# Banksylel/Restrictive-Hierarchical-Semantic-Segmentation

Hardware: AMD Instinct MI355X
Metric: train images/sec (620x620, hier-HRNet-W48) (higher is better)
Workload: dtype f32 (fp16x2 split on fp16 MFMA, 22-bit operands, fp32 accumulate; exact-fp32 MFMA on the small problems); 1 GPU; HRNet-W48 hierarchical (class_tree_tl.json), 620x620, batch 4 per GPU, train_epoch batch body (fwd L passes, prediction prep + metrics, CE+Dice+consistency, bwd, grad all-reduce, AdamW, metric vectors, one D2H readback of loss+metrics); global_batch=4, parallelism=dp1, launch=launch tape replay, rccl_ranks=1, level_passes=batched (one launch per layer for all L passes)

## Files before the change

### include/hrseg.h

```cpp
#ifndef HRSEG_H
#define HRSEG_H

#include <stddef.h>
#include <stdint.h>

#ifdef __cplusplus
extern "C" {
#endif

typedef void* hrseg_stream_t;

enum hrseg_status {
  HRSEG_OK = 0,
  HRSEG_ERR_INVALID_ARG = -1,
  HRSEG_ERR_LAUNCH = -2,
  HRSEG_ERR_UNSUPPORTED = -3,
};

const char* hrseg_last_error_string(void);
int hrseg_abi_version(void);

enum hrseg_conv_precision { HRSEG_CONV_F32 = 0, HRSEG_CONV_BF16X3 = 1, HRSEG_CONV_BF16X2 = 2, HRSEG_CONV_BF16 = 3, HRSEG_CONV_AUTO = 4,
                            HRSEG_CONV_FP16X2 = 5 };
typedef struct {
// ... 121 lines not shown
int hrseg_head_bn_fwd(const float* y, int ldy, const float* coef, const float* gb, const float* w, const float* bias,
                      float* z, int ldz, int B, long hw, int F, int Cout, hrseg_stream_t stream);
#define HRSEG_HEAD_BN_MAX_SEG 8
typedef struct {
  const float* y; int ldy; const float* coef;
  int F, nseg, B; long hw;
  double* partial; int nchunks;
  float* dy_absmax;
  float* dy; int lddy;
  const float* gb[HRSEG_HEAD_BN_MAX_SEG]; const float* w[HRSEG_HEAD_BN_MAX_SEG];
  const float* dzl[HRSEG_HEAD_BN_MAX_SEG]; int lddzl[HRSEG_HEAD_BN_MAX_SEG]; int Cout[HRSEG_HEAD_BN_MAX_SEG];
  float* dw[HRSEG_HEAD_BN_MAX_SEG]; float* dbias[HRSEG_HEAD_BN_MAX_SEG]; float* dgb[HRSEG_HEAD_BN_MAX_SEG];
} hrseg_head_bn_t;
int hrseg_head_bn_bwd_reduce(const hrseg_head_bn_t* p, int seg0, int nsegs, hrseg_stream_t stream);
int hrseg_head_bn_bwd_apply(const hrseg_head_bn_t* p, hrseg_stream_t stream);
int hrseg_logits_up_fwd(const float* in, int ldin, int B, int Hi, int Wi, int C, float* out, int Ho,
                        int Wo, int align_corners, hrseg_stream_t stream);
int hrseg_logits_up_bwd(const float* dout, int B, int Hi, int Wi, int C, float* din, int lddin,
                        int Ho, int Wo, int align_corners, hrseg_stream_t stream);

int hrseg_sigmoid_fwd(const float* z, float* p, long n, hrseg_stream_t stream);
int hrseg_compose_fwd(const float* z, const float* pprev, float* p, int B, int C, int Cprev,
                      long hw, int ngroups, const int* group_parent, const int* group_size,
                      hrseg_stream_t stream);
int hrseg_compose_bwd(const float* dp, long sb, long sc, long si, const float* z,
                      const float* pprev, float* dz, int dz_accumulate, float* dpprev,
                      int dpprev_accumulate, int B, int C, int Cprev, long hw, int ngroups,
                      const int* group_parent, const int* group_size, hrseg_stream_t stream);
int hrseg_sigmoid_bwd(const float* dp, long sb, long sc, long si, const float* z, float* dz,
                      int accumulate, int B, int C, long hw, hrseg_stream_t stream);
// ... 226 lines not shown
```

### restrictive-hierarchical-semantic-segmentation_amd/_lib.py

```python
from __future__ import annotations

import ctypes as C
import os

import torch

_HERE = os.path.dirname(os.path.abspath(__file__))
LIB_PATH = os.path.join(_HERE, "csrc", "libhrseg_hip.so")

if not os.path.exists(LIB_PATH):
    raise ImportError(
        f"{LIB_PATH} not found: the MI355X HIP library is not built. "
        "Run `make -C restrictive-hierarchical-semantic-segmentation_amd/csrc` (needs hipcc); "
        "there is no CPU fallback for the product path.")

_lib = C.CDLL(LIB_PATH)

_p = C.c_void_p
_i = C.c_int
_l = C.c_long
_f = C.c_float


class ConvShape(C.Structure):
# ... 9 lines not shown
                ("running_var", _p), ("num_batches_tracked", _p), ("momentum", _f), ("eps", _f), ("residual", _p),
                ("ldr", _i), ("relu", _i), ("z", _p), ("ldz", _i), ("coef", _p), ("partial", _p), ("nchunks", _i),
                ("stat_div", _i), ("stat_updates", _i), ("relu_mask", _p), ("z_split", _i), ("residual_split", _i), ("stat_ranks", _i)]


class BnBwd(C.Structure):
    _fields_ = [("dz", _p), ("lddz", _i), ("z", _p), ("ldz", _i), ("relu", _i), ("y", _p), ("ldy", _i), ("coef", _p),
                ("dgamma", _p), ("dbeta", _p), ("dy", _p), ("lddy", _i), ("dres", _p), ("lddres", _i),
                ("dres_accumulate", _i), ("npix", _l), ("C", _i), ("partial", _p), ("nchunks", _i), ("dy_absmax", _p), ("nseg", _i), ("relu_mask", _p), ("sum_ranks", _i)]


class HeadBn(C.Structure):
    _fields_ = [("y", _p), ("ldy", _i), ("coef", _p), ("F", _i), ("nseg", _i), ("B", _i), ("hw", _l), ("partial", _p),
                ("nchunks", _i), ("dy_absmax", _p), ("dy", _p), ("lddy", _i), ("gb", _p * 8), ("w", _p * 8), ("dzl", _p * 8),
                ("lddzl", _i * 8), ("Cout", _i * 8), ("dw", _p * 8), ("dbias", _p * 8), ("dgb", _p * 8)]


class DecodeTree(C.Structure):
    _fields_ = [("first_child", (_i * 16) * 8), ("n_children", (_i * 16) * 8), ("pixel_val", (_i * 16) * 8), ("root_softmax", _i)]


class Hedge(C.Structure):
    _fields_ = [("tau", (_f * 16) * 8), ("stop_val", (_i * 16) * 8), ("reject_val", _i)]


PROTOTYPES = {
    "hrseg_conv_fwd_group": [_i, _p, _p, _p, _p, C.POINTER(ConvShape), _p],
    "hrseg_conv_dgrad_group": [_i, _p, _p, _p, _p, C.POINTER(ConvShape), _p],
    "hrseg_conv_wgrad_group": [_i, _p, _p, _p, C.POINTER(ConvShape), _p],
    "hrseg_conv_wgrad_group_ws": [_i, _p, _p, _p, C.POINTER(ConvShape), _p, C.c_size_t, _p],
# ... 15 lines not shown
    "hrseg_weight_cols_gather": [_p, _i, _i, _i, _p, _p, _p],
    "hrseg_weight_cols_scatter_add": [_p, _i, _i, _i, _p, _p, _p],
    "hrseg_add": [_p, _i, _p, _i, _p, _i, _i, _l, _i, _p],
    "hrseg_copy": [_p, _i, _p, _i, _i, _l, _i, _p],
    "hrseg_relu_bwd": [_p, _i, _p, _i, _p, _i, _l, _i, _p],
    "hrseg_nchw_to_nhwc": [_p, _p, _i, _i, _i, _i, _i, _p],
    "hrseg_nhwc_to_nchw": [_p, _i, _p, _i, _i, _i, _i, _p],
    "hrseg_gap_nchw": [_p, _p, _p, _i, _l, _p],
    "hrseg_film_linear_fwd": [_p, _p, _p, _p, _i, _i, _i, _p],
    "hrseg_film_linear_bwd": [_p, _p, _p, _p, _p, _p, _i, _i, _i, _f, _p],
    "hrseg_head_fwd": [_p, _i, _p, _p, _p, _p, _i, _i, _l, _i, _i, _p],
    "hrseg_head_bwd": [_p, _i, _p, _p, _p, _i, _p, _i, _i, _p, _p, _p, _i, _l, _i, _i, _p],
    "hrseg_head_bn_fwd": [_p, _i, _p, _p, _p, _p, _p, _i, _i, _l, _i, _i, _p],
    "hrseg_head_bn_bwd_reduce": [C.POINTER(HeadBn), _i, _i, _p],
    "hrseg_head_bn_bwd_apply": [C.POINTER(HeadBn), _p],
    "hrseg_logits_up_fwd": [_p, _i, _i, _i, _i, _i, _p, _i, _i, _i, _p],
    "hrseg_logits_up_bwd": [_p, _i, _i, _i, _i, _p, _i, _i, _i, _i, _p],
    "hrseg_sigmoid_fwd": [_p, _p, _l, _p],
    "hrseg_sigmoid_bwd": [_p, _l, _l, _l, _p, _p, _i, _i, _i, _l, _p],
    "hrseg_compose_fwd": [_p, _p, _p, _i, _i, _i, _l, _i, _p, _p, _p],
    "hrseg_compose_bwd": [_p, _l, _l, _l, _p, _p, _p, _i, _p, _i, _i, _i, _i, _l, _i, _p, _p, _p],
    "hrseg_loss_partials": [_p, _p, _p, _i, _i, _l, _p],
    "hrseg_loss_finalize": [_p, _p, _i, _i, _p, _p, _p],
    "hrseg_loss_bwd": [_p, _p, _p, _p, _p, _i, _i, _i, _l, _p],
    "hrseg_loss_partials_opt": [_p, _p, _p, _i, _i, _l, _f, _p],
    "hrseg_loss_finalize_opt": [_p, _p, _i, _i, _f, _f, _f, _p, _p, _p],
    "hrseg_loss_bwd_opt": [_p, _p, _p, _p, _p, _i, _i, _i, _l, _f, _p],
    "hrseg_ohem_scores": [_p, _p, _p, _i, _i, _l, _p],
    "hrseg_ohem_select": [_p, _l, _f, _l, _p, _p, _p],
    "hrseg_loss_partials_ohem": [_p, _p, _p, _p, _f, _p, _i, _i, _l, _f, _p],
# ... 133 lines not shown
def launch_count(family=None, reset=False) -> int:
    return int(_lib.hrseg_launch_count(None if family is None else family.encode(), int(reset)))


def deterministic() -> bool:
    return _deterministic


_fuse_bwd_multi = True


def fuse_bwd_multi() -> bool:
    return _fuse_bwd_multi


_tune_generation = 0


def tune_generation() -> int:
    return _tune_generation


def tune(**kv):
    global _deterministic, _fuse_bwd_multi, _tune_generation
    _tune_generation += 1
    for k, v in kv.items():
        if _lib.hrseg_tune(k.encode(), int(v)) != 0:
            raise RuntimeError(f"hrseg_tune({k}) failed: {last_error()}")
        if k == "deterministic":
            _deterministic = bool(v)
        if k == "fuse_bwd_multi":
            _fuse_bwd_multi = bool(v)


def set_conv_tune(wtm=0, kc=0, db=0, ksplit=0):
    tune(igemm_wtm=wtm, igemm_kc=kc, igemm_db=db, igemm_ksplit=ksplit)


def set_wgrad_tune(pix=0, db=0, target_blocks=0):
    tune(wgrad_pix=pix, wgrad_db=db, wgrad_blocks=target_blocks)


def set_wgrad_group_plan(mult=0, min_blocks=0, max_blocks=0):
    tune(wgrad_group_mult=mult, wgrad_group_min=min_blocks, wgrad_group_max=max_blocks)


_fn = {}
# ... 207 lines not shown
```

### restrictive-hierarchical-semantic-segmentation_amd/csrc/bn.hip

```cpp
#include <type_traits>
#include "elem_common.h"
#include "sp_arith.h"

__device__ __forceinline__ void reduce_chunks16(const double* __restrict__ partial, int nchunks, int C, int c,
                                               double& s0, double& s1, double* red) {
  const int lane = threadIdx.x >> 4;
  double a = 0.0, b = 0.0;
  if (c < C) {
    int k = lane;
    for (; k + 48 < nchunks; k += 64) {
      double t0[4], t1[4];
#pragma unroll
      for (int u = 0; u < 4; ++u) {
        t0[u] = partial[((size_t)(k + 16 * u) * 2 + 0) * C + c];
        t1[u] = partial[((size_t)(k + 16 * u) * 2 + 1) * C + c];
      }
#pragma unroll
      for (int u = 0; u < 4; ++u) {
        a += t0[u];
        b += t1[u];
      }
    }
    for (; k < nchunks; k += 16) {
      a += partial[((size_t)k * 2 + 0) * C + c];
// ... 767 lines not shown
}

extern "C" int hrseg_bn_bwd_group(int n, const hrseg_bn_bwd_t* probs, int eval_mode, hrseg_stream_t stream) {
  return hrseg_bn_bwd_group_phases(n, probs, eval_mode, 7, stream);
}

extern "C" int hrseg_bn_bwd_group_phases(int n, const hrseg_bn_bwd_t* probs, int eval_mode, int phases, hrseg_stream_t stream) {
  HRSEG_CHECK_ARG(n >= 1 && n <= BN_MAXG && probs, "hrseg_bn_bwd_group: n must be 1..%d", BN_MAXG);
  HRSEG_CHECK_ARG(phases > 0 && phases <= 7, "hrseg_bn_bwd_group_phases: phases is a mask of bits 0..2");
  hipStream_t st = (hipStream_t)stream;
  BnBwdG g;
  g.h.n = n;
  for (int i = 0; i < n; ++i) {
    const hrseg_bn_bwd_t& p = probs[i];
    if (int e = check_c(p.C, "hrseg_bn_bwd_group")) return e;
    HRSEG_CHECK_ARG(p.dz && p.y && p.coef && p.dy && p.partial && p.npix > 0 && p.nchunks > 0,
                    "hrseg_bn_bwd_group: bad arguments");
    HRSEG_CHECK_ARG(p.nseg <= 1 || (p.nchunks % p.nseg == 0 && p.npix % p.nseg == 0),
                    "hrseg_bn_bwd_group: nseg=%d must divide nchunks=%d and npix", p.nseg, p.nchunks);
    if (int e = check_operand(p.dz, p.lddz, p.C, "hrseg_bn_bwd_group", "dz")) return e;
    if (int e = check_operand(p.y, p.ldy, p.C, "hrseg_bn_bwd_group", "y")) return e;
    if (int e = check_operand(p.dy, p.lddy, p.C, "hrseg_bn_bwd_group", "dy")) return e;
    if (p.relu && p.z)
      if (int e = check_operand(p.z, p.ldz, p.C, "hrseg_bn_bwd_group", "z")) return e;
    if (p.dres)
      if (int e = check_operand(p.dres, p.lddres, p.C, "hrseg_bn_bwd_group", "dres")) return e;
    HRSEG_CHECK_ARG(al16(p.coef), "hrseg_bn_bwd_group: coef must be 16-byte aligned");
    g.p[i] = p;
  }
  int end = 0;
  bool masked = false;
  for (int i = 0; i < n; ++i) masked = masked || (probs[i].relu && probs[i].relu_mask);
  if (phases & 1) {
    for (int i = 0; i < n; ++i) { end += probs[i].nchunks; g.h.blk_end[i] = end; }
    if (masked) hipLaunchKernelGGL(bn_bwd_reduce_group_kernel<true>, dim3(end), dim3(256), 0, st, g);
    else hipLaunchKernelGGL(bn_bwd_reduce_group_kernel<false>, dim3(end), dim3(256), 0, st, g);
    HRSEG_LAUNCH_CHECK("bn_bwd_reduce_group");
  }
  if (phases & 2) {
    end = 0;
    for (int i = 0; i < n; ++i) { end += ceil_div(probs[i].C, 16); g.h.blk_end[i] = end; }
    hipLaunchKernelGGL(bn_bwd_finalize_group_kernel, dim3(end), dim3(256), 0, st, g);
// ... 71 lines not shown
```

### restrictive-hierarchical-semantic-segmentation_amd/csrc/runtime.h

```cpp
#pragma once

#define HRSEG_FAMILIES(X)                   \
  X(WS, "ws", 1)                            \
  X(WS_GROUP, "ws_group", 1)                \
  X(PATCH_SP, "patch_sp", 1)                \
  X(SP_IM2COL, "sp_im2col", 1)              \
  X(SP_PGROUP, "sp_pgroup", 1)              \
  X(SP_GROUP, "sp_group", 1)                \
  X(F32, "f32", 1)                          \
  X(F32_GROUP, "f32_group", 1)              \
  X(WGRAD_SP, "wgrad_sp", 1)                \
  X(WGRAD_F32, "wgrad_f32", 1)              \
  X(WGRAD_F32_GROUP, "wgrad_f32_group", 1)  \
  X(WGRAD9, "wgrad9", 1)                    \
  X(SMALL_CIN, "small_cin", 1)              \
  X(SP_WIDE, "sp_wide", 1)                  \
  X(WS_CANVAS, "ws_canvas", 0)              \
  X(WGRAD_SP_GROUP, "wgrad_sp_group", 1)    \
  X(WGRAD_SP_T5, "wgrad_sp_t5", 0)          \
  X(WGRAD_SP_WIDE, "wgrad_sp_wide", 1)      \
  X(AUG_IMAGE, "augment_image", 0)          \
  X(AUG_TARGETS, "augment_targets", 0)      \
  X(DECODE_LABELS, "decode_labels", 0)      \
  X(SCORE_LABELS, "score_labels", 0)        \
  X(DECODE_VIEWS, "decode_views", 0)        \
  X(FLIP_VIEWS, "flip_views", 0)          \
  X(WINDOW_CROPS, "window_crops", 0)      \
  X(DECODE_WINDOWS, "decode_windows", 0)  \
  X(OHEM, "ohem", 0)                      \
  X(LABEL_COMPONENTS, "label_components", 0)  \
  X(FILTER_COMPONENTS, "filter_components", 0)  \
  X(SCORE_BOUNDARIES, "score_boundaries", 0)  \
  X(SCORE_INSTANCES, "score_instances", 0)  \
  X(SCORE_CALIBRATION, "score_calibration", 0)  \
  X(DECODE_HEDGED, "decode_hedged", 0)  \
  X(MIX, "mix", 0)  \
  X(BORDER_WEIGHTS, "border_weights", 0)
#define HRSEG_X(id, name, conv) CNT_##id,
enum { HRSEG_FAMILIES(HRSEG_X) CNT_N };
#undef HRSEG_X
extern long hrseg_g_cnt[CNT_N];
static inline void hrseg_count(int id, long n = 1) { hrseg_g_cnt[id] += n; }

#define HRSEG_KNOBS(X)                                                                                                               \
  X(igemm_wtm, 0, 0, "fp32 implicit GEMM: pixel tiles per wave (1, 2, 4; +10 = 96-channel tiles)")                                   \
  X(igemm_kc, 0, 0, "fp32 implicit GEMM: 16-channel chunks per K stage")                                                             \
  X(igemm_db, 0, 0, "fp32 implicit GEMM: LDS buffers")                                                                               \
  X(igemm_ksplit, 0, 0, "fp32 implicit GEMM: split-K factor")                                                                        \
  X(group_wtm, 0, 0, "grouped launches: pixel tile, 1 = 64, 2 = 128 pixels")                                                         \
  X(wgrad_pix, 0, 0, "weight gradient: pixels per stage")                                                                            \
  X(wgrad_db, 0, 0, "weight gradient: LDS buffers")                                                                                  \
  X(wgrad_blocks, 0, 0, "weight gradient: target grid")                                                                              \
// ... 22 lines not shown
  X(wgrad9_blocks2, 0, 0, "  ... of two")                                                                                            \
  X(wgrad9_blocks3, 0, 0, "  ... of three")                                                                                          \
  X(wgrad9_blocks4, 0, 0, "  ... of four")                                                                                           \
  X(sp_wide, 1, 0, "0 = never use the wide-tile im2col body, 2 = also on short reductions (tests)")                                  \
  X(sp_ws_canvas, 5, 0, "canvas tiling of small images: least cut of the padded area, percent (0 = per-image tiles everywhere)")     \
  X(wgrad_group_sp, 1, 0, "0 = grouped tap-per-block weight gradients stay on the fp32 kernel")                                      \
  X(wgrad_sp_t5, 1, 0, "0 = no 80 x 80 tiles in the tap-per-block weight gradient")                                                  \
  X(wgrad_sp_wide, 1, 0, "0 = never the wide-tile weight-gradient body")                                                             \
  X(sp_wide_min_blocks, 256, 0, "wide-tile im2col body: least number of 128-pixel blocks")                                           \
  X(sp_patch_min_tiles, 192, 1, "routing threshold: least tile count of the halo-patch body")                                        \
  X(auto_min_pixels, 8192, 1, "routing threshold: HRSEG_CONV_AUTO runs fp16x2 from this many output pixels on")                      \
  X(sp_ws_min_tiles, 96, 1, "routing threshold: least tile count of the wave-specialised body")                                      \
  X(deterministic, 0, 0, "1 = every float reduction with a run-dependent order takes its single-adder form (common.h)")             \
  X(bwd_multi_slab, 0, 0, "multi-target bilinear transpose: channels of a slab of the streaming body (0 = automatic, < 0 = the gather body)") \
  X(bwd_multi_bands, 0, 0, "  ... its bands of target rows per image (0 = automatic; clamped to the coarsest target's rows)")        \
  X(fuse_bwd_multi, 1, 0, "0 = the fuse layers' backward transposes each low-resolution term in a launch of its own (engine.py)")
#define HRSEG_X(key, def, restore, meaning) extern int hrseg_g_##key;
HRSEG_KNOBS(HRSEG_X)
#undef HRSEG_X
```

### restrictive-hierarchical-semantic-segmentation_amd/engine.py

```python
from __future__ import annotations

import contextlib
import os

import torch

from . import _lib, ops

_SIDE = {}


_SIDE_ENABLED = None
_RELU_MASK = os.environ.get("HRSEG_BN_RELU_MASK", "1") != "0"
_EXPERIMENT = set(filter(None, os.environ.get("HRSEG_EXPERIMENT", "").split(",")))
_CONV_STATS = os.environ.get("HRSEG_CONV_STATS", "1") != "0"
_X_SPLIT = int(os.environ.get("HRSEG_X_SPLIT", "2"))


def wgrad_stream(device):
    global _SIDE_ENABLED
    if _SIDE_ENABLED is None:
        _SIDE_ENABLED = os.environ.get("HRSEG_WGRAD_STREAM", "1") != "0"
    if not _SIDE_ENABLED:
        return None
# ... 197 lines not shown
                                  split_for=[split_for] if split_for is not None else None, defer=defer)[0]

    def conv_bn_group(self, items, relu, outs=None, single_reader=False, split_for=None, split_level=1, defer=False):
        n = len(items)
        relus = list(relu) if isinstance(relu, (list, tuple)) else [relu] * n
        k, s = items[0][1].kernel_size[0], items[0][1].stride[0]
        assert all(c.kernel_size[0] == k and c.stride[0] == s for _, c, _, _ in items)
        xs = [it[0] for it in items]
        if not self.training and not self.record and self.fold is not None:
            folded = [self.fold(conv, bn) for _, conv, bn, _ in items]
            res = [it[3].data if it[3] is not None else None for it in items]
            prec = self.prec if all(f[2] for f in folded) else _lib.CONV_PRECISION["f32"]
            zs = ops.conv_fwd_group([x.data for x in xs], [f[0] for f in folded], [f[1] for f in folded], k, s,
                                    [c.out_channels for _, c, _, _ in items], prec=prec, residuals=res, relus=relus, outs=outs)
            return [Act(z) for z in zs]
        want_stats = self.training and _CONV_STATS and self.sync is None and not _lib.deterministic() and not _EXPERIMENT
        stats = None
        ys = ops.conv_fwd_group([x.data for x in xs], [c.weight._hr_store for _, c, _, _ in items],
                                [c.bias._hr_store if c.bias is not None else None for _, c, _, _ in items], k, s,
                                [c.out_channels for _, c, _, _ in items], prec=self.prec, stats=want_stats,
                                wpersist=self.wpersist, x_splits=[x.split for x in xs])
        if want_stats:
            ys, stats = ys
        if stats is not None and any(st is None for st in stats):
            stats = None

        def conv_backward(dys, gmax_all, gmaxs):
            def weight_gradients():
                if "skip_wgrad" in _EXPERIMENT:
                    return
# ... 10 lines not shown
            while todo:
                seen, rnd, rest = set(), [], []
                for i in todo:
                    (rest if id(xs[i]) in seen else rnd).append(i)
                    seen.add(id(xs[i]))
                wp = self.wpersist and all(hasattr(items[i][1].weight, "_hr_tstore_range") for i in rnd)
                got = ops.conv_dgrad_group([dys[i] for i in rnd], [self._wt(items[i][1]) for i in rnd],
                                           [xs[i].data.shape for i in rnd], k, s, [xs[i].grad for i in rnd],
                                           [xs[i].grad is not None for i in rnd], prec=self.prec,
                                           gmaxs=[gmaxs[i] for i in rnd], wpersist=wp)
                for i, o in zip(rnd, got):
                    xs[i].grad = o
                todo = rest
        return self._bn_tail([(bn, res) for _, _, bn, res in items], ys, stats, relus, conv_backward, outs=outs,
                             single_reader=single_reader, split_for=split_for, split_level=split_level, defer=defer)

    def _keep_for_side(self, side, *tensors):
        tensors = [t for t in tensors if t is not None]
        if _lib.taping():
            _lib.tape_keep(*tensors)
        else:
            for t in tensors:
                t.record_stream(side)
        self.used_side = True

    def _bn_tail(self, bns, ys, stats, relus, backward, outs=None, single_reader=False, split_for=None, split_level=1,
                 defer=False):
        n = len(ys)
        masks = [torch.empty((y.shape[0] * y.shape[1] * y.shape[2], y.shape[3] // 4), dtype=torch.uint8, device=y.device)
                 if (self.record and _RELU_MASK and relus[i] and res is not None) else None
# ... 250 lines not shown
```

### restrictive-hierarchical-semantic-segmentation_amd/ops.py

```python
from __future__ import annotations

import ctypes as C
import os
from typing import NamedTuple

import torch

from . import _lib
from ._lib import ConvShape, call, ptr


def _ld(t):
    assert t.dim() == 4 and (t.stride(3) == 1 or t.shape[3] == 1), "NHWC tensor with contiguous channels expected"
    B, H, W, Cn = t.shape
    if W > 1:
        ld = t.stride(2)
    elif H > 1:
        ld = t.stride(1)
    elif B > 1:
        ld = t.stride(0)
    else:
        ld = Cn
    assert (H == 1 or t.stride(1) == W * ld) and (B == 1 or t.stride(0) == H * W * ld) and ld >= Cn, \
        "only channel-sliced NHWC views are supported"
# ... 1340 lines not shown
    a.dz, a.lddz, a.y, a.ldy, a.coef = ptr(y), _ld(y), ptr(y), _ld(y), ptr(coef)
    a.dy, a.lddy = ptr(y), _ld(y)
    a.dgamma, a.dbeta = ptr(dgamma), ptr(dbeta)
    a.npix, a.C, a.partial, a.nchunks, a.nseg, a.sum_ranks = _npix(y), F, ptr(partial), int(nchunks), nseg, 1
    call("hrseg_bn_bwd_group_phases", 1, arr, 0, 2)


def head_bn_bwd_apply(y, coef, nseg, partial, nchunks, heads, dy=None, dy_absmax=None):
    if dy is None:
        dy = torch.empty(y.shape, dtype=torch.float32, device=y.device)
    a = _head_bn_struct(y, coef, nseg, partial, nchunks, heads, dy=dy, dy_absmax=dy_absmax)
    call("hrseg_head_bn_bwd_apply", C.byref(a))
    return dy


def logits_up_fwd(z, Ho, Wo, align_corners=True):
    B, Hi, Wi, Cn = z.shape
    out = torch.empty((B, Cn, Ho, Wo), dtype=torch.float32, device=z.device)
    call("hrseg_logits_up_fwd", ptr(z), _ld(z), B, Hi, Wi, Cn, ptr(out), Ho, Wo, int(align_corners))
    return out


def logits_up_bwd(dout, Hi, Wi, align_corners=True):
    B, Cn, Ho, Wo = dout.shape
    din = empty_nhwc(B, Hi, Wi, Cn, dout)
    call("hrseg_logits_up_bwd", ptr(dout), B, Hi, Wi, Cn, ptr(din), Cn, Ho, Wo, int(align_corners))
    return din


def sigmoid_fwd(z):
# ... 266 lines not shown
```

Baseline: 97.03 images/s.

## Fuse the 3-channel stem conv with BatchNorm by recomputing its output

Adds dedicated stem kernels for the first 3x3 conv with three input channels. The forward pass computes BN statistics from the conv output on the fly and recomputes the conv in the apply pass, so the pre-BN conv activation is never stored. The backward pass recomputes it again for the BN reduce and the fused wgrad. This removes the full-resolution write and read of the stem activation and the generic low-channel conv path, at the cost of computing the cheap 27-tap conv three times.

After: 97.72 images/s, median of 6. Within noise of the previous version (+0.7%).

```diff
diff --git a/include/hrseg.h b/include/hrseg.h
--- a/include/hrseg.h
+++ b/include/hrseg.h
@@ -159,6 +159,23 @@
 } hrseg_head_bn_t;
 int hrseg_head_bn_bwd_reduce(const hrseg_head_bn_t* p, int seg0, int nsegs, hrseg_stream_t stream);
 int hrseg_head_bn_bwd_apply(const hrseg_head_bn_t* p, hrseg_stream_t stream);
+typedef struct {
+  const float* x; int ldx;
+  int B, Hi, Wi, Cin, Ho, Wo, ksize, stride;
+  const float* w; const float* bias; int Cout;
+  const float* residual;
+  const float* coef;
+  double* partial; int nchunks; int nseg;
+  int relu;
+  float* z; int ldz; int z_split;
+  const float* dz; int lddz;
+  float* dw;
+  float* dw_ws; int dw_ws_blocks;
+} hrseg_stem_t;
+int hrseg_stem_stats(const hrseg_stem_t* p, hrseg_stream_t stream);
+int hrseg_stem_apply(const hrseg_stem_t* p, hrseg_stream_t stream);
+int hrseg_stem_bwd_reduce(const hrseg_stem_t* p, hrseg_stream_t stream);
+int hrseg_stem_bwd_apply_wgrad(const hrseg_stem_t* p, hrseg_stream_t stream);
 int hrseg_logits_up_fwd(const float* in, int ldin, int B, int Hi, int Wi, int C, float* out, int Ho,
                         int Wo, int align_corners, hrseg_stream_t stream);
 int hrseg_logits_up_bwd(const float* dout, int B, int Hi, int Wi, int C, float* din, int lddin,
diff --git a/restrictive-hierarchical-semantic-segmentation_amd/_lib.py b/restrictive-hierarchical-semantic-segmentation_amd/_lib.py
--- a/restrictive-hierarchical-semantic-segmentation_amd/_lib.py
+++ b/restrictive-hierarchical-semantic-segmentation_amd/_lib.py
@@ -47,6 +47,12 @@
     _fields_ = [("y", _p), ("ldy", _i), ("coef", _p), ("F", _i), ("nseg", _i), ("B", _i), ("hw", _l), ("partial", _p),
                 ("nchunks", _i), ("dy_absmax", _p), ("dy", _p), ("lddy", _i), ("gb", _p * 8), ("w", _p * 8), ("dzl", _p * 8),
                 ("lddzl", _i * 8), ("Cout", _i * 8), ("dw", _p * 8), ("dbias", _p * 8), ("dgb", _p * 8)]
+
+
+class Stem(C.Structure):
+    _fields_ = [("x", _p), ("ldx", _i)] + [(n, _i) for n in ("B", "Hi", "Wi", "Cin", "Ho", "Wo", "ksize", "stride")] + \
+               [("w", _p), ("bias", _p), ("Cout", _i), ("residual", _p), ("coef", _p), ("partial", _p), ("nchunks", _i),
+                ("nseg", _i), ("relu", _i), ("z", _p), ("ldz", _i), ("z_split", _i), ("dz", _p), ("lddz", _i), ("dw", _p), ("dw_ws", _p), ("dw_ws_blocks", _i)]
 
 
 class DecodeTree(C.Structure):
@@ -92,6 +98,10 @@
     "hrseg_head_bn_fwd": [_p, _i, _p, _p, _p, _p, _p, _i, _i, _l, _i, _i, _p],
     "hrseg_head_bn_bwd_reduce": [C.POINTER(HeadBn), _i, _i, _p],
     "hrseg_head_bn_bwd_apply": [C.POINTER(HeadBn), _p],
+    "hrseg_stem_stats": [C.POINTER(Stem), _p],
+    "hrseg_stem_apply": [C.POINTER(Stem), _p],
+    "hrseg_stem_bwd_reduce": [C.POINTER(Stem), _p],
+    "hrseg_stem_bwd_apply_wgrad": [C.POINTER(Stem), _p],
     "hrseg_logits_up_fwd": [_p, _i, _i, _i, _i, _i, _p, _i, _i, _i, _p],
     "hrseg_logits_up_bwd": [_p, _i, _i, _i, _i, _p, _i, _i, _i, _i, _p],
     "hrseg_sigmoid_fwd": [_p, _p, _l, _p],
@@ -255,6 +265,13 @@
     return _fuse_bwd_multi
 
 
+_stem_knobs = {"stem_fuse": True, "small_cin3": True}
+
+
+def stem_fuse() -> bool:
+    return all(_stem_knobs.values())
+
+
 _tune_generation = 0
 
 
@@ -272,6 +289,8 @@
             _deterministic = bool(v)
         if k == "fuse_bwd_multi":
             _fuse_bwd_multi = bool(v)
+        if k in _stem_knobs:
+            _stem_knobs[k] = bool(v)
 
 
 def set_conv_tune(wtm=0, kc=0, db=0, ksplit=0):
diff --git a/restrictive-hierarchical-semantic-segmentation_amd/csrc/bn.hip b/restrictive-hierarchical-semantic-segmentation_amd/csrc/bn.hip
--- a/restrictive-hierarchical-semantic-segmentation_amd/csrc/bn.hip
+++ b/restrictive-hierarchical-semantic-segmentation_amd/csrc/bn.hip
@@ -805,18 +805,24 @@
   for (int i = 0; i < n; ++i) {
     const hrseg_bn_bwd_t& p = probs[i];
     if (int e = check_c(p.C, "hrseg_bn_bwd_group")) return e;
-    HRSEG_CHECK_ARG(p.dz && p.y && p.coef && p.dy && p.partial && p.npix > 0 && p.nchunks > 0,
-                    "hrseg_bn_bwd_group: bad arguments");
+    const bool reduce = phases & 1, apply = phases & 4;
+    HRSEG_CHECK_ARG(p.partial && p.npix > 0 && p.nchunks > 0, "hrseg_bn_bwd_group: bad arguments");
+    HRSEG_CHECK_ARG(!(reduce || apply) || (p.dz && p.y && p.coef), "hrseg_bn_bwd_group: bad arguments");
+    HRSEG_CHECK_ARG(!apply || p.dy, "hrseg_bn_bwd_group: bad arguments");
     HRSEG_CHECK_ARG(p.nseg <= 1 || (p.nchunks % p.nseg == 0 && p.npix % p.nseg == 0),
                     "hrseg_bn_bwd_group: nseg=%d must divide nchunks=%d and npix", p.nseg, p.nchunks);
-    if (int e = check_operand(p.dz, p.lddz, p.C, "hrseg_bn_bwd_group", "dz")) return e;
-    if (int e = check_operand(p.y, p.ldy, p.C, "hrseg_bn_bwd_group", "y")) return e;
-    if (int e = check_operand(p.dy, p.lddy, p.C, "hrseg_bn_bwd_group", "dy")) return e;
-    if (p.relu && p.z)
-      if (int e = check_operand(p.z, p.ldz, p.C, "hrseg_bn_bwd_group", "z")) return e;
-    if (p.dres)
-      if (int e = check_operand(p.dres, p.lddres, p.C, "hrseg_bn_bwd_group", "dres")) return e;
-    HRSEG_CHECK_ARG(al16(p.coef), "hrseg_bn_bwd_group: coef must be 16-byte aligned");
+    if (reduce || apply) {
+      if (int e = check_operand(p.dz, p.lddz, p.C, "hrseg_bn_bwd_group", "dz")) return e;
+      if (int e = check_operand(p.y, p.ldy, p.C, "hrseg_bn_bwd_group", "y")) return e;
+      if (p.relu && p.z)
+        if (int e = check_operand(p.z, p.ldz, p.C, "hrseg_bn_bwd_group", "z")) return e;
+      HRSEG_CHECK_ARG(al16(p.coef), "hrseg_bn_bwd_group: coef must be 16-byte aligned");
+    }
+    if (apply) {
+      if (int e = check_operand(p.dy, p.lddy, p.C, "hrseg_bn_bwd_group", "dy")) return e;
+      if (p.dres)
+        if (int e = check_operand(p.dres, p.lddres, p.C, "hrseg_bn_bwd_group", "dres")) return e;
+    }
     g.p[i] = p;
   }
   int end = 0;
diff --git a/restrictive-hierarchical-semantic-segmentation_amd/csrc/runtime.h b/restrictive-hierarchical-semantic-segmentation_amd/csrc/runtime.h
--- a/restrictive-hierarchical-semantic-segmentation_amd/csrc/runtime.h
+++ b/restrictive-hierarchical-semantic-segmentation_amd/csrc/runtime.h
@@ -35,7 +35,8 @@
   X(SCORE_CALIBRATION, "score_calibration", 0)  \
   X(DECODE_HEDGED, "decode_hedged", 0)  \
   X(MIX, "mix", 0)  \
-  X(BORDER_WEIGHTS, "border_weights", 0)
+  X(BORDER_WEIGHTS, "border_weights", 0)  \
+  X(STEM_FUSED, "stem_fused", 0)
 #define HRSEG_X(id, name, conv) CNT_##id,
 enum { HRSEG_FAMILIES(HRSEG_X) CNT_N };
 #undef HRSEG_X
@@ -88,7 +89,8 @@
   X(deterministic, 0, 0, "1 = every float reduction with a run-dependent order takes its single-adder form (common.h)")             \
   X(bwd_multi_slab, 0, 0, "multi-target bilinear transpose: channels of a slab of the streaming body (0 = automatic, < 0 = the gather body)") \
   X(bwd_multi_bands, 0, 0, "  ... its bands of target rows per image (0 = automatic; clamped to the coarsest target's rows)")        \
-  X(fuse_bwd_multi, 1, 0, "0 = the fuse layers' backward transposes each low-resolution term in a launch of its own (engine.py)")
+  X(fuse_bwd_multi, 1, 0, "0 = the fuse layers' backward transposes each low-resolution term in a launch of its own (engine.py)") \
+  X(stem_fuse, 1, 0, "0 = the first layer keeps its stored convolution output: the hrseg_stem_* entry points refuse (stem.hip, engine.py)")
 #define HRSEG_X(key, def, restore, meaning) extern int hrseg_g_##key;
 HRSEG_KNOBS(HRSEG_X)
 #undef HRSEG_X
diff --git a/restrictive-hierarchical-semantic-segmentation_amd/csrc/stem.hip b/restrictive-hierarchical-semantic-segmentation_amd/csrc/stem.hip
--- /dev/null
+++ b/restrictive-hierarchical-semantic-segmentation_amd/csrc/stem.hip
@@ -0,0 +1,463 @@
+#include "elem_common.h"
+#include "sp_arith.h"
+
+#define STEM_TILE 64
+
+struct StemK {
+  const float* x; int ldx, Hi, Wi, Ho, Wo, stride;
+  const float* w; const float* bias; int C;
+  const float* coef; double* partial; int nchunks, nseg;
+  long npix;
+  int relu; float* z; int ldz, z_split;
+  const float* dz; int lddz;
+  float* dw; int pix_per_block;
+  float* dw_ws;
+};
+
+struct PixPos { int b, oy, ox; };
+__device__ __forceinline__ PixPos pix_pos(int m, int Ho, int Wo) {
+  PixPos p;
+  const int hw = Ho * Wo;
+  p.b = m / hw;
+  const int rem = m - p.b * hw;
+  p.oy = rem / Wo;
+  p.ox = rem - p.oy * Wo;
+  return p;
+}
+__device__ __forceinline__ void pix_advance(PixPos& p, int n, int Ho, int Wo) {
+  p.ox += n;
+  while (p.ox >= Wo) {
+    p.ox -= Wo;
+    if (++p.oy == Ho) {
+      p.oy = 0;
+      ++p.b;
+    }
+  }
+}
+
+struct TapRegs { float v[3][3]; };
+__device__ __forceinline__ void tap_fetch(const StemK& a, const PixPos& at, int s0, int hi, int np, TapRegs& r) {
+#pragma unroll
+  for (int i = 0; i < 3; ++i) {
+    const int j = threadIdx.x + 256 * i;
+    r.v[i][0] = r.v[i][1] = r.v[i][2] = 0.f;
+    const int pp = j / 9, t = j - pp * 9;
+    if (pp < np && s0 + pp < hi) {
+      PixPos q = at;
+      pix_advance(q, pp, a.Ho, a.Wo);
+      const int iy = q.oy * a.stride + t / 3 - 1, ix = q.ox * a.stride + t % 3 - 1;
+      if ((unsigned)iy < (unsigned)a.Hi && (unsigned)ix < (unsigned)a.Wi) {
+        const float* xp = a.x + ((size_t)(q.b * a.Hi + iy) * a.Wi + ix) * a.ldx;
+        r.v[i][0] = xp[0];
+        r.v[i][1] = xp[1];
+        r.v[i][2] = xp[2];
+      }
+    }
+  }
+}
+__device__ __forceinline__ void tap_commit(float (*xs)[9][4], int np, const TapRegs& r) {
+#pragma unroll
+  for (int i = 0; i < 3; ++i) {
+    const int j = threadIdx.x + 256 * i;
+    const int pp = j / 9, t = j - pp * 9;
+    if (pp < np) *reinterpret_cast<f32x4*>(&xs[pp][t][0]) = f32x4{r.v[i][0], r.v[i][1], r.v[i][2], 0.f};
+  }
+}
+
+__device__ __forceinline__ void load_quad_weights(const float* __restrict__ w, int co, float (&wr)[27][4]) {
+  const float* base = w + (size_t)co * 27;
+#pragma unroll
+  for (int i = 0; i < 27; ++i) {
+    const f32x4 v = ld4(base + 4 * i);
+#pragma unroll
+    for (int e = 0; e < 4; ++e) wr[(4 * i + e) % 27][(4 * i + e) / 27] = v[e];
+  }
+}
+
+__device__ __forceinline__ f32x4 stem_y4(const float (*xt)[4], const float (&wr)[27][4], f32x4 bv) {
+  f32x4 acc = {0.f, 0.f, 0.f, 0.f};
+#pragma unroll
+  for (int t = 0; t < 9; ++t) {
+    const f32x4 xv = *reinterpret_cast<const f32x4*>(&xt[t][0]);
+#pragma unroll
+    for (int ci = 0; ci < 3; ++ci)
+#pragma unroll
+      for (int j = 0; j < 4; ++j) acc[j] = fmaf(xv[ci], wr[t * 3 + ci][j], acc[j]);
+  }
+  return acc + bv;
+}
+
+__device__ __forceinline__ void chunk_range(long npix, int nchunks, int nseg, int chunk, int& lo, int& hi) {
+  const int cps = nchunks / nseg, seg = chunk / cps;
+  const long seg_pix = npix / nseg;
+  const long per = (seg_pix + cps - 1) / cps;
+  const long l = seg * seg_pix + (long)(chunk - seg * cps) * per;
+  const long seg_end = (seg + 1) * seg_pix;
+  const long h = (l + per < seg_end) ? l + per : seg_end;
+  lo = (int)(l < h ? l : h);
+  hi = (int)h;
+}
+
+__device__ __forceinline__ void write_partials(const Lanes& L, int C, f32x4 s, f32x4 s2, double* red, double* __restrict__ partial, int chunk) {
+#pragma unroll
+  for (int j = 0; j < 4; ++j) {
+    red[threadIdx.x * 8 + j] = s[j];
+    red[threadIdx.x * 8 + 4 + j] = s2[j];
+  }
+  __syncthreads();
+  for (int c = threadIdx.x; c < C; c += 256) {
+    double sa = 0.0, sb = 0.0;
+    for (int pl = 0; pl < L.P; ++pl) {
+      const int t = pl * L.Q + (c >> 2);
+      sa += red[t * 8 + (c & 3)];
+      sb += red[t * 8 + 4 + (c & 3)];
+    }
+    partial[((size_t)chunk * 2 + 0) * C + c] = sa;
+    partial[((size_t)chunk * 2 + 1) * C + c] = sb;
+  }
+}
+
+template <bool BWD>
+__global__ __launch_bounds__(256) void stem_sums_kernel(StemK a) {
+  __shared__ double red[256 * 8];
+  __shared__ __attribute__((aligned(16))) float xs[STEM_TILE][9][4];
+  const int C = a.C;
+  const Lanes L = make_lanes(C);
+  const int np = 4 * L.P;
+  const int chunk = blockIdx.x;
+  int lo, hi;
+  chunk_range(a.npix, a.nchunks, BWD ? a.nseg : 1, chunk, lo, hi);
+  const int cq = L.active ? L.cq : 0;
+  float wr[27][4];
+  load_quad_weights(a.w, 4 * cq, wr);
+  f32x4 bv = {0.f, 0.f, 0.f, 0.f};
+  if (a.bias) bv = ld4(a.bias + 4 * cq);
+  f32x4 mean = {0.f, 0.f, 0.f, 0.f}, rstd = {1.f, 1.f, 1.f, 1.f}, sc = mean, sh = mean;
+  if (BWD) {
+    mean = ld4(a.coef + 4 * cq);
+    rstd = ld4(a.coef + C + 4 * cq);
+    sc = ld4(a.coef + 2 * C + 4 * cq);
+    sh = ld4(a.coef + 3 * C + 4 * cq);
+  }
+  const f32x4 zero = {0.f, 0.f, 0.f, 0.f};
+  f32x4 s = zero, s2 = zero;
+  TapRegs tr;
+  f32x4 gn[4];
+  auto fetch_dz = [&](int s0) {
+#pragma unroll
+    for (int u = 0; u < 4; ++u) {
+      const int pix = s0 + L.pl + u * L.P;
+      gn[u] = (L.active && pix < hi) ? ld4(a.dz + (size_t)pix * a.lddz + 4 * cq) : zero;
+    }
+  };
+  PixPos at = {0, 0, 0};
+  if (lo < hi) {
+    at = pix_pos(lo, a.Ho, a.Wo);
+    tap_fetch(a, at, lo, hi, np, tr);
+    if (BWD) fetch_dz(lo);
+  }
+  for (int s0 = lo; s0 < hi; s0 += np) {
+    __syncthreads();
+    tap_commit(xs, np, tr);
+    __syncthreads();
+    f32x4 g[4];
+    if (BWD) {
+#pragma unroll
+      for (int u = 0; u < 4; ++u) g[u] = gn[u];
+    }
+    if (s0 + np < hi) {
+      pix_advance(at, np, a.Ho, a.Wo);
+      tap_fetch(a, at, s0 + np, hi, np, tr);
+      if (BWD) fetch_dz(s0 + np);
+    }
+    if (L.active) {
+#pragma unroll
+      for (int u = 0; u < 4; ++u) {
+        const int pp = L.pl + u * L.P;
+        const bool ok = s0 + pp < hi;
+        if (!BWD) {
+          const f32x4 v = ok ? stem_y4(xs[pp], wr, bv) : zero;
+          s += v;
+          s2 += v * v;
+        } else {
+          const f32x4 yv = ok ? stem_y4(xs[pp], wr, bv) : mean;
+          f32x4 gv = g[u];
+          if (a.relu) {
+            const f32x4 zc = bn_affine(yv, sc, sh);
+#pragma unroll
+            for (int j = 0; j < 4; ++j) gv[j] = zc[j] > 0.f ? gv[j] : 0.f;
+          }
+          const f32x4 xh = (yv - mean) * rstd;
+          s += gv;
+          s2 += gv * xh;
+        }
+      }
+    }
+  }
+  write_partials(L, C, s, s2, red, a.partial, chunk);
+}
+
+__global__ __launch_bounds__(256) void stem_apply_kernel(StemK a, int tiles_per_block) {
+  __shared__ __attribute__((aligned(16))) float xs[STEM_TILE][9][4];
+  const int C = a.C;
+  const Lanes L = make_lanes(C);
+  const int np = 4 * L.P;
+  const int cq = L.active ? L.cq : 0;
+  float wr[27][4];
+  load_quad_weights(a.w, 4 * cq, wr);
+  f32x4 bv = {0.f, 0.f, 0.f, 0.f};
+  if (a.bias) bv = ld4(a.bias + 4 * cq);
+  const f32x4 sc = ld4(a.coef + 2 * C + 4 * cq), sh = ld4(a.coef + 3 * C + 4 * cq);
+  const int npix = (int)a.npix;
+  const long l = (long)blockIdx.x * tiles_per_block * np;
+  const int lo = (int)(l < npix ? l : npix);
+  const int hi = (int)(l + (long)tiles_per_block * np < npix ? l + (long)tiles_per_block * np : npix);
+  TapRegs tr;
+  PixPos at = {0, 0, 0};
+  if (lo < hi) {
+    at = pix_pos(lo, a.Ho, a.Wo);
+    tap_fetch(a, at, lo, hi, np, tr);
+  }
+  for (int s0 = lo; s0 < hi; s0 += np) {
+    __syncthreads();
+    tap_commit(xs, np, tr);
+    __syncthreads();
+    if (s0 + np < hi) {
+      pix_advance(at, np, a.Ho, a.Wo);
+      tap_fetch(a, at, s0 + np, hi, np, tr);
+    }
+    if (L.active) {
+#pragma unroll
+      for (int u = 0; u < 4; ++u) {
+        const int pp = L.pl + u * L.P;
+        const int pix = s0 + pp;
+        if (pix < hi) {
+          f32x4 v = bn_affine(stem_y4(xs[pp], wr, bv), sc, sh);
+          if (a.relu) v = relu_nan(v);
+          if (a.z_split) *reinterpret_cast<u32x4*>(a.z + (size_t)pix * a.ldz + 4 * cq) = hrseg_split_f16x2(v);
+          else st4(a.z + (size_t)pix * a.ldz + 4 * cq, v);
+        }
+      }
+    }
+  }
+}
+
+__global__ __launch_bounds__(256) void stem_bwd_wgrad_kernel(StemK a) {
+  constexpr int P = 64;
+  __shared__ __attribute__((aligned(16))) float dzs[P][64];
+  __shared__ __attribute__((aligned(16))) float xs[P][9][4];
+  __shared__ float red[3][64][28];
+  const int tid = threadIdx.x;
+  const int C = a.C, co0 = blockIdx.y * 64, co = co0 + (tid & 63), col = tid & 63, pg = tid >> 6;
+  const int M = (int)a.npix;
+  const int lo = blockIdx.x * a.pix_per_block;
+  const int hi = a.pix_per_block < M - lo ? lo + a.pix_per_block : M;
+  float wr[27];
+#pragma unroll
+  for (int k = 0; k < 27; ++k) wr[k] = a.w[(size_t)co * 27 + k];
+  const float bv = a.bias ? a.bias[co] : 0.f;
+  const float mean = a.coef[co], rstd = a.coef[C + co], scale = a.coef[2 * C + co], shift = a.coef[3 * C + co];
+  const double* totals = a.partial + (size_t)a.nchunks * 2 * C;
+  const int nseg = a.nseg;
+  const int seg_pix = M / nseg;
+  const float inv = (float)(1.0 / (double)seg_pix);
+  int seg_end = lo;
+  float mg = 0.f, mgx = 0.f;
+  float acc[9][3];
+#pragma unroll
+  for (int t = 0; t < 9; ++t)
+#pragma unroll
+    for (int c = 0; c < 3; ++c) acc[t][c] = 0.f;
+  TapRegs tr;
+  f32x4 gn[(P * 16) / 256];
+  auto fetch_dz = [&](int s0) {
+#pragma unroll
+    for (int r = 0; r < (P * 16) / 256; ++r) {
+      const int j = tid + 256 * r;
+      const int m = s0 + (j >> 4);
+      gn[r] = m < hi ? ld4(a.dz + (size_t)m * a.lddz + co0 + (j & 15) * 4) : f32x4{0.f, 0.f, 0.f, 0.f};
+    }
+  };
+  PixPos at = pix_pos(lo, a.Ho, a.Wo);
+  tap_fetch(a, at, lo, hi, P, tr);
+  fetch_dz(lo);
+  for (int s0 = lo; s0 < hi; s0 += P) {
+    __syncthreads();
+    tap_commit(xs, P, tr);
+#pragma unroll
+    for (int r = 0; r < (P * 16) / 256; ++r) {
+      const int j = tid + 256 * r;
+      st4(&dzs[j >> 4][(j & 15) * 4], gn[r]);
+    }
+    __syncthreads();
+    if (s0 + P < hi) {
+      pix_advance(at, P, a.Ho, a.Wo);
+      tap_fetch(a, at, s0 + P, hi, P, tr);
+      fetch_dz(s0 + P);
+    }
+#pragma unroll 2
+    for (int q = 0; q < P / 4; ++q) {
+      const int pp = pg * (P / 4) + q;
+      const int m = s0 + pp;
+      f32x4 xv[9];
+#pragma unroll
+      for (int t = 0; t < 9; ++t) xv[t] = *reinterpret_cast<const f32x4*>(&xs[pp][t][0]);
+      float dyv = 0.f;
+      if (m < hi) {
+        if (m >= seg_end) {
+          const int seg = m / seg_pix;
+          seg_end = (seg + 1) * seg_pix;
+          mg = (float)(totals[(size_t)seg * 2 * C + co]) * inv;
+          mgx = (float)(totals[(size_t)seg * 2 * C + C + co]) * inv;
+        }
+        float y = 0.f;
+#pragma unroll
+        for (int t = 0; t < 9; ++t)
+#pragma unroll
+          for (int c = 0; c < 3; ++c) y = fmaf(xv[t][c], wr[t * 3 + c], y);
+        const float yv = y + bv;
+        float gg = dzs[pp][col];
+        if (a.relu) {
+          const float zz = __builtin_fmaf(yv, scale, shift);
+          gg = zz > 0.f ? gg : 0.f;
+        }
+        const float xh = (yv - mean) * rstd;
+        dyv = scale * (gg - mg - xh * mgx);
+      }
+#pragma unroll
+      for (int t = 0; t < 9; ++t)
+#pragma unroll
+        for (int c = 0; c < 3; ++c) acc[t][c] = fmaf(dyv, xv[t][c], acc[t][c]);
+    }
+  }
+  if (pg > 0) {
+#pragma unroll
+    for (int t = 0; t < 9; ++t)
+#pragma unroll
+      for (int c = 0; c < 3; ++c) red[pg - 1][col][t * 3 + c] = acc[t][c];
+  }
+  __syncthreads();
+  if (pg == 0) {
+#pragma unroll
+    for (int t = 0; t < 9; ++t)
+#pragma unroll
+      for (int c = 0; c < 3; ++c) {
+        const float v = ((acc[t][c] + red[0][col][t * 3 + c]) + red[1][col][t * 3 + c]) + red[2][col][t * 3 + c];
+        if (a.dw_ws) a.dw_ws[((size_t)blockIdx.x * C + co) * 27 + t * 3 + c] = v;
+        else atomicAdd(a.dw + ((size_t)co * 9 + t) * 3 + c, v);
+      }
+  }
+}
+
+__global__ __launch_bounds__(256) void stem_dw_reduce_kernel(const float* __restrict__ ws, float* __restrict__ dw, int n, int nblk) {
+  __shared__ float red[16][17];
+  const int wi = threadIdx.x & 15, l = threadIdx.x >> 4;
+  const int i = blockIdx.x * 16 + wi;
+  float s = 0.f;
+  if (i < n)
+    for (int k = l; k < nblk; k += 16) s += ws[(size_t)k * n + i];
+  red[l][wi] = s;
+  __syncthreads();
+  if (l == 0 && i < n) {
+    float t = red[0][wi];
+    for (int q = 1; q < 16; ++q) t += red[q][wi];
+    dw[i] += t;
+  }
+}
+
+static int check_stem(const hrseg_stem_t* p, const char* who, StemK& k) {
+  HRSEG_CHECK_ARG(p, "%s: NULL problem", who);
+  if (!hrseg_g_stem_fuse) {
+    hrseg_set_error("%s: switched off (hrseg_tune stem_fuse = 0): use hrseg_conv_fwd_group + hrseg_bn_fwd_group", who);
+    return HRSEG_ERR_UNSUPPORTED;
+  }
+  HRSEG_CHECK_ARG(p->Cin == 3 && p->ksize == 3 && (p->stride == 1 || p->stride == 2),
+                  "%s: Cin=%d ksize=%d stride=%d: only the 3-channel 3x3 layer at stride 1 or 2", who, p->Cin, p->ksize, p->stride);
+  HRSEG_CHECK_ARG(p->Cout > 0 && p->Cout % 64 == 0 && p->Cout <= 1024, "%s: Cout=%d must be a multiple of 64 and <= 1024", who, p->Cout);
+  HRSEG_CHECK_ARG(p->B > 0 && p->Hi > 0 && p->Wi > 0 && p->Ho == (p->Hi - 1) / p->stride + 1 && p->Wo == (p->Wi - 1) / p->stride + 1,
+                  "%s: output %dx%d does not match input %dx%d k3 s%d", who, p->Ho, p->Wo, p->Hi, p->Wi, p->stride);
+  HRSEG_CHECK_ARG((long)p->B * p->Ho * p->Wo < (1L << 31) && (long)p->B * p->Hi * p->Wi < (1L << 31), "%s: 2^31 pixels or more", who);
+  HRSEG_CHECK_ARG(p->residual == nullptr, "%s: a layer with a residual keeps the separate launches", who);
+  HRSEG_CHECK_ARG(p->x && p->w, "%s: null pointer", who);
+  HRSEG_CHECK_ARG(p->ldx >= 3 && (uintptr_t)p->x % 4 == 0, "%s: bad image (ldx=%d)", who, p->ldx);
+  HRSEG_CHECK_ARG(al16(p->w) && (!p->bias || al16(p->bias)), "%s: w and bias must be 16-byte aligned", who);
+  k.x = p->x; k.ldx = p->ldx; k.Hi = p->Hi; k.Wi = p->Wi; k.Ho = p->Ho; k.Wo = p->Wo; k.stride = p->stride;
+  k.w = p->w; k.bias = p->bias; k.C = p->Cout;
+  k.coef = p->coef; k.partial = p->partial; k.nchunks = p->nchunks; k.nseg = p->nseg > 1 ? p->nseg : 1;
+  k.npix = (long)p->B * p->Ho * p->Wo;
+  k.relu = p->relu; k.z = p->z; k.ldz = p->ldz; k.z_split = p->z_split;
+  k.dz = p->dz; k.lddz = p->lddz; k.dw = p->dw; k.pix_per_block = 0; k.dw_ws = nullptr;
+  return 0;
+}
+static int check_stem_coef(const hrseg_stem_t* p, const char* who) {
+  HRSEG_CHECK_ARG(p->coef && al16(p->coef), "%s: coef must be given, 16-byte aligned", who);
+  return 0;
+}
+static int check_stem_sums(const hrseg_stem_t* p, const StemK& k, const char* who) {
+  HRSEG_CHECK_ARG(p->partial && p->nchunks > 0, "%s: partial / nchunks", who);
+  HRSEG_CHECK_ARG(k.nseg == 1 || (p->nchunks % k.nseg == 0 && k.npix % k.nseg == 0), "%s: nseg=%d must divide nchunks=%d and the pixel count",
+                  who, k.nseg, p->nchunks);
+  return 0;
+}
+
+extern "C" int hrseg_stem_stats(const hrseg_stem_t* p, hrseg_stream_t stream) {
+  StemK k;
+  if (int e = check_stem(p, "hrseg_stem_stats", k)) return e;
+  k.nseg = 1;
+  if (int e = check_stem_sums(p, k, "hrseg_stem_stats")) return e;
+  hipLaunchKernelGGL(stem_sums_kernel<false>, dim3(k.nchunks), dim3(256), 0, (hipStream_t)stream, k);
+  hrseg_count(CNT_STEM_FUSED);
+  HRSEG_LAUNCH_CHECK("stem_stats");
+  return 0;
+}
+
+extern "C" int hrseg_stem_apply(const hrseg_stem_t* p, hrseg_stream_t stream) {
+  StemK k;
+  if (int e = check_stem(p, "hrseg_stem_apply", k)) return e;
+  if (int e = check_stem_coef(p, "hrseg_stem_apply")) return e;
+  HRSEG_CHECK_ARG(p->z, "hrseg_stem_apply: null pointer");
+  if (int e = check_operand(p->z, p->ldz, p->Cout, "hrseg_stem_apply", "z")) return e;
+  const int Q = k.C / 4, np = 4 * (Q >= 256 ? 1 : 256 / Q);
+  const int ntiles = ceil_div(k.npix, np);
+  const int tpb = ntiles >= 8 * 2048 ? ceil_div(ntiles, 2048) : ntiles >= 8 * 512 ? 8 : ceil_div(ntiles, 512);
+  hipLaunchKernelGGL(stem_apply_kernel, dim3(ceil_div(ntiles, tpb)), dim3(256), 0, (hipStream_t)stream, k, tpb);
+  hrseg_count(CNT_STEM_FUSED);
+  HRSEG_LAUNCH_CHECK("stem_apply");
+  return 0;
+}
+
+extern "C" int hrseg_stem_bwd_reduce(const hrseg_stem_t* p, hrseg_stream_t stream) {
+  StemK k;
+  if (int e = check_stem(p, "hrseg_stem_bwd_reduce", k)) return e;
+  if (int e = check_stem_coef(p, "hrseg_stem_bwd_reduce")) return e;
+  if (int e = check_stem_sums(p, k, "hrseg_stem_bwd_reduce")) return e;
+  HRSEG_CHECK_ARG(p->dz, "hrseg_stem_bwd_reduce: null pointer");
+  if (int e = check_operand(p->dz, p->lddz, p->Cout, "hrseg_stem_bwd_reduce", "dz")) return e;
+  hipLaunchKernelGGL(stem_sums_kernel<true>, dim3(k.nchunks), dim3(256), 0, (hipStream_t)stream, k);
+  hrseg_count(CNT_STEM_FUSED);
+  HRSEG_LAUNCH_CHECK("stem_bwd_reduce");
+  return 0;
+}
+
+extern "C" int hrseg_stem_bwd_apply_wgrad(const hrseg_stem_t* p, hrseg_stream_t stream) {
+  StemK k;
+  if (int e = check_stem(p, "hrseg_stem_bwd_apply_wgrad", k)) return e;
+  if (int e = check_stem_coef(p, "hrseg_stem_bwd_apply_wgrad")) return e;
+  if (int e = check_stem_sums(p, k, "hrseg_stem_bwd_apply_wgrad")) return e;
+  HRSEG_CHECK_ARG(p->dz && p->dw, "hrseg_stem_bwd_apply_wgrad: null pointer");
+  if (int e = check_operand(p->dz, p->lddz, p->Cout, "hrseg_stem_bwd_apply_wgrad", "dz")) return e;
+  HRSEG_CHECK_ARG((uintptr_t)p->dw % 4 == 0, "hrseg_stem_bwd_apply_wgrad: dw must be 4-byte aligned");
+  const int nblk_target = hrseg_g_deterministic ? 1 : hrseg_g_wgrad_blocks ? hrseg_g_wgrad_blocks : 512;
+  k.pix_per_block = ceil_div(ceil_div(k.npix, nblk_target), 64) * 64;
+  const int nblk = ceil_div(k.npix, k.pix_per_block);
+  const bool ws = p->dw_ws && nblk <= p->dw_ws_blocks;
+  if (ws) {
+    HRSEG_CHECK_ARG((uintptr_t)p->dw_ws % 4 == 0, "hrseg_stem_bwd_apply_wgrad: dw_ws must be 4-byte aligned");
+    k.dw_ws = p->dw_ws;
+  }
+  hipLaunchKernelGGL(stem_bwd_wgrad_kernel, dim3(nblk, k.C / 64), dim3(256), 0, (hipStream_t)stream, k);
+  if (ws) hipLaunchKernelGGL(stem_dw_reduce_kernel, dim3(ceil_div(27 * k.C, 16)), dim3(256), 0, (hipStream_t)stream, k.dw_ws, k.dw, 27 * k.C, nblk);
+  hrseg_count(CNT_STEM_FUSED);
+  HRSEG_LAUNCH_CHECK("stem_bwd_apply_wgrad");
+  return 0;
+}
diff --git a/restrictive-hierarchical-semantic-segmentation_amd/engine.py b/restrictive-hierarchical-semantic-segmentation_amd/engine.py
--- a/restrictive-hierarchical-semantic-segmentation_amd/engine.py
+++ b/restrictive-hierarchical-semantic-segmentation_amd/engine.py
@@ -235,6 +235,10 @@
             zs = ops.conv_fwd_group([x.data for x in xs], [f[0] for f in folded], [f[1] for f in folded], k, s,
                                     [c.out_channels for _, c, _, _ in items], prec=prec, residuals=res, relus=relus, outs=outs)
             return [Act(z) for z in zs]
+        if n == 1 and not defer and (outs is None or outs[0] is None):
+            fused = self.stem_conv_bn(items[0], relus[0], split_for[0] if split_for is not None else None, split_level)
+            if fused is not None:
+                return [fused]
         want_stats = self.training and _CONV_STATS and self.sync is None and not _lib.deterministic() and not _EXPERIMENT
         stats = None
         ys = ops.conv_fwd_group([x.data for x in xs], [c.weight._hr_store for _, c, _, _ in items],
@@ -275,6 +279,37 @@
                 todo = rest
         return self._bn_tail([(bn, res) for _, _, bn, res in items], ys, stats, relus, conv_backward, outs=outs,
                              single_reader=single_reader, split_for=split_for, split_level=split_level, defer=defer)
+
+    def stem_conv_bn(self, item, relu, split_for=None, split_level=1):
+        x, conv, bn, res = item
+        if not (self.training and res is None and self.sync is None and not _lib.deterministic() and not _EXPERIMENT):
+            return None
+        if x.needs_grad or x.split or os.environ.get("HRSEG_STEM_FUSE", "1") == "0" or not _lib.stem_fuse():
+            return None
+        k, s, cout = conv.kernel_size[0], conv.stride[0], conv.out_channels
+        if not (conv.in_channels == 3 and x.data.shape[3] == 3 and k == 3 and conv.padding[0] == 1 and s in (1, 2) and cout % 64 == 0
+                and cout <= 1024 and conv.dilation[0] == 1 and conv.groups == 1 and bn.track_running_stats):
+            return None
+        xd = x.data
+        B, Hi, Wi, _ = xd.shape
+        z_split = False
+        if split_for is not None and _X_SPLIT >= split_level:
+            zshape = (B, ops.conv_out_size(Hi, k, s), ops.conv_out_size(Wi, k, s), cout)
+            z_split = ops.conv_x_split_ok([zshape], [split_for.out_channels], split_for.kernel_size[0], split_for.stride[0], self.prec)
+        w, bias = conv.weight._hr_store, (conv.bias._hr_store if conv.bias is not None else None)
+        z, coef, _ = ops.stem_fwd(xd, w, bias, cout, k, s,
+                                  dict(gamma=bn.weight._hr_store, beta=bn.bias._hr_store, rm=bn.running_mean, rv=bn.running_var,
+                                       nbt=bn.num_batches_tracked, momentum=bn.momentum, eps=bn.eps, repeat=self.bn_repeat,
+                                       stat_div=self.bn_segments), relu, z_split=z_split)
+        out = Act(z, split=z_split)
+        if self.record:
+            def bwd():
+                dz = out.grad
+                out.grad = None
+                ops.stem_bwd(xd, w, bias, cout, k, s, dz, coef, relu, bn.weight._hr_gstore, bn.bias._hr_gstore,
+                             conv.weight._hr_gstore, nseg=self.bn_segments)
+            self._push(bwd)
+        return out
 
     def _keep_for_side(self, side, *tensors):
         tensors = [t for t in tensors if t is not None]
diff --git a/restrictive-hierarchical-semantic-segmentation_amd/ops.py b/restrictive-hierarchical-semantic-segmentation_amd/ops.py
--- a/restrictive-hierarchical-semantic-segmentation_amd/ops.py
+++ b/restrictive-hierarchical-semantic-segmentation_amd/ops.py
@@ -1378,6 +1378,64 @@
     return dy
 
 
+def _stem_struct(x, w, bias, cout, k, s, residual=None):
+    B, Hi, Wi, Cin = x.shape
+    a = _lib.Stem()
+    a.x, a.ldx, a.B, a.Hi, a.Wi, a.Cin = ptr(x), _ld(x), B, Hi, Wi, Cin
+    a.Ho, a.Wo, a.ksize, a.stride = conv_out_size(Hi, k, s), conv_out_size(Wi, k, s), k, s
+    a.w, a.bias, a.Cout, a.residual = ptr(w), ptr(bias), int(cout), ptr(residual)
+    return a
+
+
+STEM_WS_BLOCKS = 512
+
+
+def stem_chunks(npix, cout, nseg=1):
+    nch = _nchunks(npix, cout)
+    return max(nseg, nch // nseg * nseg) if nseg > 1 else nch
+
+
+def stem_fwd(x, w, bias, cout, k, s, bn, relu, z_split=False, out=None, residual=None):
+    a = _stem_struct(x, w, bias, cout, k, s, residual)
+    npix = a.B * a.Ho * a.Wo
+    nch = stem_chunks(npix, cout)
+    part = torch.empty(nch * 2 * cout, dtype=torch.float64, device=x.device)
+    coef = torch.empty(4 * cout, dtype=torch.float32, device=x.device)
+    z = out if out is not None else torch.empty((a.B, a.Ho, a.Wo, cout), dtype=torch.float32, device=x.device)
+    a.partial, a.nchunks, a.nseg = ptr(part), nch, 1
+    call("hrseg_stem_stats", C.byref(a))
+    arr = (_lib.BnFwd * 1)()
+    f = arr[0]
+    f.y, f.ldy, f.npix, f.C = None, 0, npix, int(cout)
+    f.gamma, f.beta, f.running_mean, f.running_var = ptr(bn["gamma"]), ptr(bn["beta"]), ptr(bn["rm"]), ptr(bn["rv"])
+    f.num_batches_tracked, f.momentum, f.eps = ptr(bn["nbt"]), float(bn["momentum"]), float(bn["eps"])
+    f.stat_updates, f.stat_div, f.stat_ranks = int(bn.get("repeat", 1)), int(bn.get("stat_div", 1)), 1
+    f.coef, f.partial, f.nchunks = ptr(coef), ptr(part), nch
+    call("hrseg_bn_fwd_group_phases", 1, arr, 1, 2)
+    a.coef, a.relu, a.z, a.ldz, a.z_split = ptr(coef), int(bool(relu)), ptr(z), _ld(z), int(bool(z_split))
+    call("hrseg_stem_apply", C.byref(a))
+    return z, coef, part
+
+
+def stem_bwd(x, w, bias, cout, k, s, dz, coef, relu, dgamma, dbeta, dw, nseg=1):
+    a = _stem_struct(x, w, bias, cout, k, s)
+    npix = a.B * a.Ho * a.Wo
+    nch = stem_chunks(npix, cout, nseg)
+    part = torch.empty((nch + nseg) * 2 * cout, dtype=torch.float64, device=x.device)
+    a.coef, a.partial, a.nchunks, a.nseg, a.relu = ptr(coef), ptr(part), nch, int(nseg), int(bool(relu))
+    a.dz, a.lddz, a.dw = ptr(dz), _ld(dz), ptr(dw)
+    ws = torch.empty(STEM_WS_BLOCKS * cout * 27, dtype=torch.float32, device=x.device)
+    a.dw_ws, a.dw_ws_blocks = ptr(ws), STEM_WS_BLOCKS
+    call("hrseg_stem_bwd_reduce", C.byref(a))
+    arr = (_lib.BnBwd * 1)()
+    b = arr[0]
+    b.coef, b.dgamma, b.dbeta = ptr(coef), ptr(dgamma), ptr(dbeta)
+    b.npix, b.C, b.partial, b.nchunks, b.nseg, b.sum_ranks = npix, int(cout), ptr(part), nch, int(nseg), 1
+    call("hrseg_bn_bwd_group_phases", 1, arr, 0, 2)
+    call("hrseg_stem_bwd_apply_wgrad", C.byref(a))
+    return part
+
+
 def logits_up_fwd(z, Ho, Wo, align_corners=True):
     B, Hi, Wi, Cn = z.shape
     out = torch.empty((B, Cn, Ho, Wo), dtype=torch.float32, device=z.device)
```
